# corelab-src/dacapo

Hardware: AMD Instinct MI355X
Metric: NTT/s (NTT-equivalents over one run() of the ResNet HEVM program, nt=2^14) (higher is better)
Workload: dtype u64; 1 GPU; ResNet-20 (SiLU) HEVM program traced from the reference's examples/benchmarks/ResNet.py with its resnet20.silu.model weights, nt=2^14 slots, N=2^15, 14 x 60-bit primes (SEAL_HEVM.cpp:39-53); one independent ciphertext stream per GPU; streams_per_gpu=1, parallelism=replicas x1 (no collective in the op path)

## Files before the change

### dacapo_amd/csrc/fused_ks.hip

```cpp
#include "ks_mac.hpp"

namespace dacapo {

struct SrcStrided {
    const u64 *base;
    long stride;
    int prime_base, period;
    __device__ int prime(int z) const { return prime_base + z % period; }
    __device__ u64 load(int z, int g, int) const { return base[(long)z * stride + g]; }
};
template <int E>
__device__ __forceinline__ void rs_operand(u64 (&v)[E], const int (&g)[E], const RsItem &it, const SumSrc *__restrict__ srcs, int p, int i,
                                           size_t N, const DModulus &M)
{
    if (it.count == 0) {
        const u64 *x = it.src.limb(p, i, N);
#pragma unroll
        for (int j = 0; j < E; j++) v[j] = x[g[j]];
    } else {
        u64 s[E];
        Acc128 a[E];
#pragma unroll
        for (int j = 0; j < E; j++) s[j] = 0, a[j].clear();
        int n_plain = 0, n_prod = 0;
// ... 173 lines not shown
                                                                              const DModulus *__restrict__ mods,
                                                                              const u64 *__restrict__ half_mod,
                                                                              const u64 *__restrict__ tw, const u64 *__restrict__ itw,
                                                                              int logN, const u64 *__restrict__ tw2)
{
    __shared__ __attribute__((aligned(16))) u64 lds[TileGeo<LOGE>::LDS_ELEMS];
    const int z = blockIdx.y, bp = MERGE ? z : z / cnt;
    const size_t N = (size_t)1 << logN;
    const u64 *in = last + (long)bp * last_stride;
    u64 x[1 << LOGE];
    auto nost = [](int, u64) {};
    ntt_tile_x<K, LOGE, true, true, true, false, true>(
        x, mods[l], itw + ((size_t)l << logN), logN, blockIdx.x, [=](int g) { return in[g]; }, nost, lds);
    const u64 ql = mods[l].q, half = ql >> 1;
#pragma unroll
    for (int r = 0; r < (1 << LOGE); r++) {
        const u64 y = x[r] + half;
        x[r] = y >= ql ? y - ql : y;
    }
    auto nold = [](int) -> u64 { return 0; };
    for (int i = MERGE ? 0 : z % cnt; i < (MERGE ? cnt : z % cnt + 1); i++) {
        u64 *out = tmp + ((size_t)bp * cnt + i) * N;
        const DModulus Mi = mods[i];
        const u64 qi = Mi.q, neg_half = qi - half_mod[(size_t)l * Kp + i];
        u64 y[1 << LOGE];
#pragma unroll
        for (int r = 0; r < (1 << LOGE); r++) {
            const u64 v = recanon(x[r], Mi) + neg_half;
            y[r] = v >= qi ? v - qi : v;
        }
        __syncthreads();
        ntt_tile_fcols<K, LOGE, false, true, false>(
            y, Mi, tw + ((size_t)i << logN), tw2 ? tw2 + ((size_t)i << (K + 1)) : nullptr, logN, blockIdx.x, nold, [=](int g, u64 v) { out[g] = v; }, lds);
    }
}

template <int K, int LOGE, bool MERGE>
__global__ __launch_bounds__(kTileThreads) void f_dr2_icols_lift_fcols_kernel(const u64 *__restrict__ acc, const MulRsItem *__restrict__ items,
                                                                               u64 *__restrict__ tmp, int ell, int Kp,
                                                                               const DModulus *__restrict__ mods,
                                                                               const u64 *__restrict__ half_mod,
                                                                               const u64 *__restrict__ inv_last, const u64 *__restrict__ tw,
                                                                               const u64 *__restrict__ itw, int logN, const u64 *__restrict__ tw2)
{
    __shared__ __attribute__((aligned(16))) u64 lds[TileGeo<LOGE>::LDS_ELEMS];
    constexpr int E = 1 << LOGE;
    const int cnt = ell - 1, L = ell - 1, sp = Kp - 1;
    const int z = blockIdx.y, bp = MERGE ? z : z / cnt;
    const size_t N = (size_t)1 << logN;
    const u64 *in_p = acc + ((size_t)bp * (ell + 1) + ell) * N, *in_l = acc + ((size_t)bp * (ell + 1) + L) * N;
    const u64 *mul = items[bp >> 1].mul;
    const long mul_stride = items[bp >> 1].mul_stride;
    auto nost = [](int, u64) {};
    u64 rho[E], u[E];
    ntt_tile_x<K, LOGE, true, true, true, false, true>(
        rho, mods[sp], itw + ((size_t)sp << logN), logN, blockIdx.x, [=](int g) { return in_p[g]; }, nost, lds);
    __syncthreads();
    const DModulus ML = mods[L];
    ntt_tile_x<K, LOGE, true, true, true, false, true>(
        u, ML, itw + ((size_t)L << logN), logN, blockIdx.x, [=](int g) { return in_l[g]; }, nost, lds);
    {
        const u64 P = mods[sp].q, half_p = P >> 1, qL = ML.q, half_l = qL >> 1;
        const u64 neg_half = qL - half_mod[(size_t)sp * Kp + L];
        u64 k = inv_last[(size_t)sp * Kp + L];
        if (mul) k = mulmod(mul[(long)L * mul_stride], k, ML);
#pragma unroll
// ... 727 lines not shown
#define DC_MERGED_LAUNCH(limbs, sources, per_source, KERNEL, ...)                                                                          \
    {                                                                                                                                     \
        const bool tiny = use_tiny_tiles(c.N, (limbs)), small = !tiny && use_small_tiles(c.N, (limbs));                                  \
        const int le = tiny ? 1 : small ? 2 : 3;                                                                                          \
        const bool merge = (per_source) > 1 && (long)(c.N >> (le == 1 ? TileGeo<1>::LOG : le == 2 ? TileGeo<2>::LOG : TileGeo<3>::LOG)) * (sources) >= ks_merge_lift_min_wgs(); \
        if (!merge) {                                                                                                                     \
            DC_GEO_SWITCH(c.k1, (limbs), DC_LAUNCH((KERNEL<KK, LE, false>), grid, dim3(kTileThreads), 0, s, __VA_ARGS__));      \
        } else if (le == 1) {                                                                                                             \
            constexpr int LE = 1;                                                                                                         \
            const dim3 grid((unsigned)(c.N >> TileGeo<LE>::LOG), (unsigned)(sources));                                                    \
            DC_K_SWITCH(c.k1, DC_LAUNCH((KERNEL<KK, LE, true>), grid, dim3(kTileThreads), 0, s, __VA_ARGS__))                    \
        } else if (le == 2) {                                                                                                             \
            constexpr int LE = 2;                                                                                                         \
            const dim3 grid((unsigned)(c.N >> TileGeo<LE>::LOG), (unsigned)(sources));                                                    \
            DC_K_SWITCH(c.k1, DC_LAUNCH((KERNEL<KK, LE, true>), grid, dim3(kTileThreads), 0, s, __VA_ARGS__))                    \
        } else {                                                                                                                          \
            constexpr int LE = 3;                                                                                                         \
            const dim3 grid((unsigned)(c.N >> TileGeo<LE>::LOG), (unsigned)(sources));                                                    \
            DC_K_SWITCH(c.k1, DC_LAUNCH((KERNEL<KK, LE, true>), grid, dim3(kTileThreads), 0, s, __VA_ARGS__))                    \
        }                                                                                                                                 \
    }

void f_ks_icols_lift_fcols(const Context &c, const u64 *digits, u64 *ext, int B, int ell, hipStream_t s)
{
    DC_MERGED_LAUNCH(B * ell * ell, B * ell, ell, f_ks_icols_lift_fcols_kernel, digits, ext, ell, c.K - 1, c.d_mods, c.d_tw, c.d_itw, c.logN, c.twc2())
}

void f_dr_icols_lift_fcols(const Context &c, const u64 *last, long last_stride, u64 *tmp, int polys, int cnt, int l, hipStream_t s)
{
    DC_MERGED_LAUNCH(polys * cnt, polys, cnt, f_dr_icols_lift_fcols_kernel, last, last_stride, tmp, cnt, l, c.K, c.d_mods, c.d_half_mod, c.d_tw,
                     c.d_itw, c.logN, c.twc2())
}

void f_dr2_icols_lift_fcols(const Context &c, const u64 *acc, const MulRsItem *items, u64 *tmp, int B, int ell, hipStream_t s)
{
    DC_MERGED_LAUNCH(2 * B * (ell - 1), 2 * B, ell - 1, f_dr2_icols_lift_fcols_kernel, acc, items, tmp, ell, c.K, c.d_mods, c.d_half_mod, c.d_inv_last,
                     c.d_tw, c.d_itw, c.logN, c.twc2())
}
#undef DC_MERGED_LAUNCH

void f_frows_fold_final(const Context &c, const u64 *tmp, const MulRsItem *items, const u64 *acc, int B, int ell, hipStream_t s, const Handoff &h)
{
    const int cnt = ell - 1, groups = h.cont == CONT_BOOT ? B : 2 * B;
#define DC_FOLD(CT)                                                                                                                    \
    DC_GEO_SWITCH(c.k2, groups * cnt, DC_LAUNCH((f_frows_fold_final_kernel<KK, LE, CT>), grid, dim3(kTileThreads), 0, s, tmp, items, acc, ell, c.K, \
                                                         c.d_mods, c.d_inv_last, c.d_tw, c.d_itw, c.logN, h))
    switch (h.cont) {
    case CONT_NONE: DC_FOLD(CONT_NONE); break;
    case CONT_MUL: DC_FOLD(CONT_MUL); break;
    case CONT_BOOT: DC_FOLD(CONT_BOOT); break;
    default: fprintf(stderr, "[dacapo_amd] f_frows_fold_final: no continuation kernel for consumer kind %d\n", h.cont); abort();
    }
#undef DC_FOLD
}

void f_ks_lift_fcols(const Context &c, const u64 *digits, u64 *ext, int B, int ell, hipStream_t s)
{
    if ((c.k1 == 7 || c.k1 == 8) && use_wide_tiles(c.N, (long)B * ell * ell) && !use_small_tiles(c.N, (long)B * ell * ell)) {
        constexpr int LE = 4;
        const dim3 grid((unsigned)(c.N >> TileGeo<LE>::LOG), (unsigned)(B * ell * ell));
        if (c.k1 == 7)
            DC_LAUNCH((f_ks_lift_fcols_kernel<7, LE>), grid, dim3(kTileThreads), 0, s, digits, ext, ell, c.K - 1, c.d_mods, c.d_tw, c.logN, c.twc2());
        else
            DC_LAUNCH((f_ks_lift_fcols_kernel<8, LE>), grid, dim3(kTileThreads), 0, s, digits, ext, ell, c.K - 1, c.d_mods, c.d_tw, c.logN, c.twc2());
        return;
    }
// ... 49 lines not shown
```

### dacapo_amd/csrc/hevm_vm.hip

```cpp
#include "hevm_vm.hpp"

#include "../../include/dacapo_ckks.h"
#include "c_api_types.hpp"
#include "chacha.hpp"
#include "seal_serial.hpp"

#include <math.h>
#include <string.h>
#include <sys/random.h>

#include <algorithm>
#include <cmath>
#include <chrono>
#include <fstream>
#include <iostream>

namespace dacapo {

constexpr int kVmThreads = 256;

constexpr int kRngCoefs = 8;

__device__ __forceinline__ int rng_cbd(u64 w)
{
// ... 33 lines not shown
            if (r[e] >= q) r[e] = w[e] >> sh;
    }
    u64x2 *o = reinterpret_cast<u64x2 *>(out + (size_t)i * N + blk * kRngCoefs);
#pragma unroll
    for (int e = 0; e < kRngCoefs; e += 2) o[e >> 1] = u64x2{ r[e], r[e + 1] };
}

__global__ __launch_bounds__(kVmThreads) void sample_small_kernel(u64 *__restrict__ out, size_t N, int limbs, int cbd, ChaChaKey key,
                                                                   u64 object, u32 domain, const DModulus *__restrict__ mods)
{
    const size_t blk = (size_t)blockIdx.x * kVmThreads + threadIdx.x;
    u64 w[kRngCoefs];
    rng_words8(key, object, blk, 0, 0, domain, w);
    int v[kRngCoefs];
#pragma unroll
    for (int e = 0; e < kRngCoefs; e++) v[e] = cbd ? rng_cbd(w[e]) : rng_ternary(w[e]);
    for (int i = 0; i < limbs; i++) store_small8(out + (size_t)i * N + blk * kRngCoefs, v, mods[i].q);
}

__global__ __launch_bounds__(kVmThreads) void sample_enc_batch_kernel(u64 *__restrict__ out, size_t N, int cnt, ChaChaKey key, u64 object0,
                                                                       const DModulus *__restrict__ mods,
                                                                       const u64 *__restrict__ epoch)
{
    const int b = blockIdx.y / 3, z = blockIdx.y % 3;
    const size_t blk = (size_t)blockIdx.x * kVmThreads + threadIdx.x;
    u64 w[kRngCoefs];
    rng_words8(key, object0 + (u64)b, blk, *epoch, 0, RNG_ENC_U + (u32)z, w);
    int v[kRngCoefs];
#pragma unroll
    for (int e = 0; e < kRngCoefs; e++) v[e] = z ? rng_cbd(w[e]) : rng_ternary(w[e]);
    for (int i = 0; i < cnt; i++) store_small8(out + (((size_t)b * 3 + z) * cnt + i) * N + blk * kRngCoefs, v, mods[i].q);
}

__global__ void chacha_blocks_kernel(u32 *__restrict__ out, ChaChaKey key, u64 counter, u64 nonce, int blocks)
{
    const int b = blockIdx.x * blockDim.x + threadIdx.x;
    if (b >= blocks) return;
    u32 o[16];
    chacha20_block(key, counter + (u64)b, nonce, o);
    for (int i = 0; i < 16; i++) out[b * 16 + i] = o[i];
}

__global__ void bump_epoch_kernel(u64 *epoch) { *epoch += 1; }

__global__ __launch_bounds__(kVmThreads) void lift_i128_kernel(u64 *__restrict__ out, const u64 *__restrict__ lo,
                                                                const u64 *__restrict__ hi, size_t N,
                                                                const DModulus *__restrict__ mods)
{
    const int i = blockIdx.y;
    const DModulus M = mods[i];
    const size_t k = (size_t)blockIdx.x * kVmThreads + threadIdx.x;
    u64 l = lo[k], h = hi[k];
    const bool neg = (h >> 63) != 0;
    if (neg) {
        l = ~l + 1;
        h = ~h + (l == 0);
    }
    const u64 r = reduce128_any(h, l, M);
    out[(size_t)i * N + k] = neg ? negmod(r, M.q) : r;
}

__global__ __launch_bounds__(kVmThreads) void ezs_final_kernel(u64 *__restrict__ c0, const u64 *__restrict__ c1,
                                                                const u64 *__restrict__ sk, const u64 *__restrict__ newkey,
                                                                int digit_lo, int digit_hi, const u64 *__restrict__ pmod, size_t N,
                                                                const DModulus *__restrict__ mods)
{
// ... 241 lines not shown
    int ksp = std::max(1, (int)option(OPT_KS_SPECIAL));
    int alpha = option(OPT_KS_ALPHA) > 0 ? (int)option(OPT_KS_ALPHA) : ksp;
    if (dir_ksp > 0) {
        if ((ksp != 1 || alpha != 1) && (ksp != dir_ksp || alpha != dir_alpha)) {
            fprintf(stderr, "[dacapo_amd] the key directory was written with ks_special = %d, ks_alpha = %d; options ask for %d / %d\n", dir_ksp,
                    dir_alpha, ksp, alpha);
            abort();
        }
        ksp = dir_ksp, alpha = dir_alpha;
    }
    ks_hoist = option(OPT_KS_HOIST) != 0;
    if (ks_hoist && (ksp > 1 || alpha > 1)) {
        fprintf(stderr, "[dacapo_amd] option ks_hoist = 1 is for SEAL-layout keys (ks_special = 1); with ks_special = %d, ks_alpha = %d key switching uses "
                        "grouped digits, which already shares a source's decomposition among its hops\n", ksp, alpha);
        abort();
    }
    ks_lazy = (int)option(OPT_KS_LAZY_SUM);
    if (ks_lazy && (ksp > 1 || alpha > 1)) {
        fprintf(stderr, "[dacapo_amd] option ks_lazy_sum = %d is for SEAL-layout keys (ks_special = 1); with ks_special = %d, ks_alpha = %d the lazy sums "
                        "of grouped-digit key switching are options hyb_lazy_sum / hyb_double_hoist\n", ks_lazy, ksp, alpha);
        abort();
    }
    if (ks_lazy && !ks_hoist) {
        fprintf(stderr, "[dacapo_amd] option ks_lazy_sum = %d needs ks_hoist = 1: a lazy sum is defined on digits taken before the automorphism "
                        "(ks_hoist = 0 here)\n", ks_lazy);
        abort();
    }
    ks_fold_rescale = option(OPT_KS_FOLD_RESCALE) != 0;
    if (ks_fold_rescale && (ksp > 1 || alpha > 1)) {
        fprintf(stderr, "[dacapo_amd] option ks_fold_rescale = 1 is for SEAL-layout keys (ks_special = 1); with ks_special = %d, ks_alpha = %d the mod-down "
                        "is an approximate base conversion, and dividing by P q in one exact pass does not reproduce it\n", ksp, alpha);
        abort();
    }
    const int bits = (int)option(OPT_PRIME_BITS);
    ctx.reset(new Context(logN, K, bits, primes, ksp, alpha));
    ctx->ensure_scratch();
    encoder.reset(new HostEncoder(logN));
    use_plan = option(OPT_PLAN) != 0;
    plan_graph = option(OPT_PLAN_GRAPH) != 0;
    plan_dag = option(OPT_PLAN_GRAPH) == 2;
    plan_lanes = option(OPT_PLAN_LANES) >= 2 ? 2 : 1;
    host_encoder = option(OPT_HOST_ENCODER) != 0;
    fold_rescale_into_boot = option(OPT_FOLD_RESCALE_BOOT) != 0;
    lazy_sums = option(OPT_HYB_LAZY_SUM) != 0;
    double_hoist = (lazy_sums && option(OPT_HYB_DOUBLE_HOIST) != 0) || ks_lazy == 2;
    max_batch = std::max(1, (int)option(OPT_MAX_BATCH));
    chain_fusion = option(OPT_CHAIN_FUSION) != 0;
    secret_weight = (int)option(OPT_SECRET_HW);
    boot_secret_weight = (int)option(OPT_BOOT_SECRET_HW);
    rot_compose = option(OPT_ROT_COMPOSE) != 0;
    online_encode = option(OPT_ONLINE_ENCODE) != 0 && use_plan && !host_encoder;
    lanes.resize(1);
    DC_HIP_CHECK(hipStreamCreateWithFlags(&lanes[0].stream, hipStreamNonBlocking));
    lanes[0].ws = ctx->ws0;
    lanes[0].boot_plain.d = dalloc((size_t)ctx->max_level() * ctx->N);
    lanes[0].boot_plain.level = ctx->max_level();
    DC_HIP_CHECK(vm_malloc(&d_epoch, 8));
    DC_HIP_CHECK(hipMemset(d_epoch, 0, 8));
    cur = 0;
}

void HEVM::gen_kswitch_key(u64 *key, const u64 *new_key, u64 key_id) { gen_kswitch_key_in(*ctx, key, keys.sk, new_key, key_id); }

void HEVM::gen_kswitch_key_in(Context &c, u64 *key, const u64 *key_sk, const u64 *new_key, u64 key_id)
{
    const size_t N = c.N;
// ... 1215 lines not shown
{
    Context &c = *ctx;
    const size_t N = c.N;
    if (!keys.sk || !keys.pk || ell < 1 || target_level < 1 || target_level > c.max_level()) {
        fprintf(stderr, "[dacapo_amd] bootstrap: needs a full VM (secret + public key) and a valid target level\n");
        abort();
    }
    const double new_scale = pow(2.0, (double)(int64_t)std::log2(src_scale));
    const CrtTables &tb = crt_tables(ell);
    u64 *pt = W().ks_tmp;
    u64 *lohi = W().ks_digits;
    f_irows_decrypt(c, src, keys.sk, ell, pt, S());
    launch_ntt_cols_inv(c, pt, (long)N, ell, nullptr, 0, 0, S());
    const CrtDev cd{ tb.inv, tb.mmod, tb.hmod, tb.hdig, tb.mdbl };
    DC_LAUNCH(reencode_kernel, dim3((unsigned)((N / 2 + kVmThreads) / kVmThreads)), dim3(kVmThreads), 0, S(), lohi,
                       lohi + N, pt, ell, N, c.d_mods, cd, new_scale / src_scale);
    Plain ptx{ lanes[cur].boot_plain.d, target_level, new_scale };
    DC_LAUNCH(lift_i128_kernel, dim3((unsigned)(N / kVmThreads), (unsigned)target_level), dim3(kVmThreads), 0, S(),
                       ptx.d, lohi, lohi + N, N, c.d_mods);
    launch_ntt(c, false, ptx.d, (long)N, target_level, nullptr, 0, 0, S());
    encrypt_plain(dst, ptx);
}

void HEVM::plan_zero_encrypt(int first, int B, int t, hipStream_t s)
{
    Context &c = *ctx;
    const size_t N = c.N;
    const int cnt = t + 1;
    if (!keys.pk) {
        fprintf(stderr, "[dacapo_amd] bootstrap: this VM has no public key\n");
        abort();
    }
    Plan &P = plan;
    DC_LAUNCH(sample_enc_batch_kernel, dim3((unsigned)(N / (kRngCoefs * kVmThreads)), (unsigned)(3 * B)), dim3(kVmThreads), 0, s,
                       P.boot_ue, N, cnt, rng.secret, ((u64)1 << 32) + (u64)first, c.d_mods, d_epoch);
    launch_ntt(c, false, P.boot_ue, (long)N, 3 * cnt * B, nullptr, 0, cnt, s);
    DC_LAUNCH(pk_encrypt_batch_kernel, dim3((unsigned)(N / (2 * kVmThreads)), (unsigned)cnt, (unsigned)(2 * B)), dim3(kVmThreads),
                       0, s, P.boot_tmp, keys.pk, (long)c.K * (long)N, P.boot_ue, cnt, N, c.d_mods);
    b_rescale(c, P.ws[0], P.d_boot_rs + first, B, cnt, s);
}

void HEVM::plan_boot_step(int first, int B, int ell, int t, int lane, hipStream_t s, const Handoff &h)
{
    Context &c = *ctx;
    const size_t N = c.N;
    if (!keys.sk) {
        fprintf(stderr, "[dacapo_amd] bootstrap: needs a full VM (secret + public key)\n");
        abort();
    }
    Plan &P = plan;
    const BootItem *items = P.d_boot + first;
    const CrtTables &tb = crt_tables(ell);
    const CrtDev cd{ tb.inv, tb.mmod, tb.hmod, tb.hdig, tb.mdbl };
    u64 *pt = P.boot_pt[lane], *ptx = P.boot_ptx[lane];
    if (h.in)
        pt = const_cast<u64 *>(h.in);
    else
        f_irows_decrypt_items(c, items, P.d_sum_srcs, keys.sk, ell, pt, B, s);
    launch_ntt_cols_inv(c, pt, (long)N, B * ell, nullptr, 0, ell, s);
    if (ell == 1)
        f_boot_reencode_fcols(c, pt, ptx, items, B, ell, t, cd, s);
    else {
        DC_LAUNCH(reencode_lift_batch_kernel, dim3((unsigned)((N / 2 + kVmThreads) / kVmThreads), (unsigned)B), dim3(kVmThreads), 0,
                           s, ptx, pt, items, ell, t, N, c.d_mods, cd);
        launch_ntt_cols_fwd(c, ptx, (long)N, B * t, nullptr, 0, t, s);
    }
// ... 436 lines not shown
```

### dacapo_amd/csrc/hevm_vm.hpp

```cpp
#pragma once
#include "wire_parse.hpp"
#include <complex>
#include <deque>
#include <map>
#include <set>
#include <memory>
#include <string>
#include <unordered_set>
#include <vector>

#include "../../include/hevm_abi.h"
#include "chacha.hpp"
#include "seal_serial.hpp"
#include "kernels.hpp"
#include "encoder.hpp"
#include "plan.hpp"

namespace dacapo {

struct VmAllocs {
    std::unordered_set<void *> live;
};
extern thread_local VmAllocs *g_vm_allocs;
template <class T>
// ... 141 lines not shown
        bool fold_rs = false;
        int gfirst = 0, gcount = 0;
        int unique = 0;
        std::vector<const u64 *> reads, writes;
    };
    struct Plan {
        bool ready = false;
        std::vector<Val> vals;
        std::vector<Pop> pops;
        std::vector<Step> steps;
        std::vector<int> final_val;
        KsItem *d_ks = nullptr;
        MulItem *d_mul = nullptr;
        MulRsItem *d_mulrs = nullptr;
        RsItem *d_rs = nullptr;
        EwItem *d_ew = nullptr;
        SumItem *d_sum = nullptr;
        SumSrc *d_sum_srcs = nullptr;
        SumGroup *d_sumg = nullptr;
        SumGroupSrc *d_sumg_srcs = nullptr;
        CtView *d_cont_other = nullptr;
        struct EncGroup { int wave, level, first, count; u64 *out; };
        std::vector<EncGroup> enc_groups;
        EncItem *d_enc_items = nullptr;
        u64 *enc_arena = nullptr;
        double2 *enc_scratch = nullptr;
        int *d_enc_overflow = nullptr;
        size_t enc_arena_bytes = 0, enc_scratch_bytes = 0;
        std::vector<EwItem> h_ew;
        std::vector<u64 *> handoff_bufs;
        size_t n_fused = 0;
        BootItem *d_boot = nullptr;
        RsItem *d_boot_rs = nullptr;
        size_t zenc_bytes = 0;
        u64 *zenc = nullptr, *boot_ue = nullptr, *boot_tmp = nullptr, *boot_pt[2] = { nullptr, nullptr }, *boot_ptx[2] = { nullptr, nullptr };
        struct BootChunk { int first, count, target; };
        std::vector<BootChunk> boot_chunks;
        BatchWs ws[2];
        std::vector<hipEvent_t> events;
        std::vector<u64 *> pool;
        int64_t n_keyswitch = 0, n_ntt = 0;
        int64_t n_hops = 0, n_decomp = 0;
        int64_t n_fold = 0;
        size_t launches = 0, max_live = 0;
        hipGraph_t graph = nullptr;
        hipGraphExec_t graph_exec = nullptr;
    } plan;
    bool plan_graph = true;
    bool plan_dag = false;
    void capture_plan();
    bool capture_plan_dag();
    void issue_step(const Step &st, hipStream_t q);
    void drop_plan_graph();
    void issue_plan(hipStream_t s);
    bool use_plan = true;
    bool test_zero_enc = false;
    int max_batch = 64;
    std::vector<u64 *> home;
    int streams = 1, sel = 0;
    std::vector<u64 *> reg_base;
    void set_streams(int n);
    void select_stream(int s);
    void build_plan();
    void run_plan();
    void boot_item(CtView src, int src_level, double src_scale, hevm_ctxt &dst, int target_level);
    void plan_zero_encrypt(int first, int B, int t, hipStream_t s);
    void plan_boot_step(int first, int B, int ell, int t, int lane, hipStream_t s, const Handoff &h);
    bool rot_compose = false;
    std::vector<int> compose_rotation(int steps) const;
    mutable std::vector<int> rot_offsets;
    mutable std::set<int> rot_offset_set;
    mutable size_t rot_offsets_epoch = (size_t)-1;
    int boot_secret_weight = 0;
    int secret_weight = 0;
    bool ks_hoist = false;
    int ks_lazy = 0;
    bool ks_fold_rescale = false;
    KsItem *d_hoist_items = nullptr;
    void rotate_hop_vm(CtView dst, CtView src, u32 elt, const u64 *key, int ell);
    bool chain_fusion = true;
    hipStream_t aux_stream = nullptr;
    bool double_hoist = false;
    double *dh_consts = nullptr;
    std::map<int, EncItem> dh_items;
    void ensure_special_limbs(const std::vector<int> &plain_regs);
    bool lazy_sums = false;
    bool fold_rescale_into_boot = false;
    int plan_lanes = 2;
    void bump_epoch(hipStream_t s);

    int64_t op_counts[11] = { 0 };
    int64_t n_keyswitch = 0, n_ntt = 0;
    int64_t n_hops = 0, n_decomp = 0;
    int64_t n_fold = 0;
    double t_bootstrap = 0.0;

    VmAllocs allocs;
    HEVM() { g_vm_allocs = &allocs; }
    void destroy_device_state();
    size_t key_elems() const { return (size_t)ctx->key_digits() * 2 * ctx->K * ctx->N; }
    void init_context(int logN, int K, const u64 *primes, int dir_ksp = 0, int dir_alpha = 0);
    void generate_keys(const RngKeys &rng, bool secret, bool pub, bool eval);
    void gen_kswitch_key(u64 *key, const u64 *new_key, u64 key_id);
    void gen_kswitch_key_in(Context &c, u64 *key, const u64 *key_sk, const u64 *new_key, u64 key_id);
    void fill_sparse_secret(u64 *dst, int weight, u32 domain);
    void generate_boot_switch_keys();
    size_t swk_down_elems() const { return (size_t)2 * (1 + ctx->ksp) * ctx->N; }
    void add_galois_key(u32 elt);
    void save_keys(const std::string &dir);
    void load_keys(const std::string &dir, bool need_secret, bool need_public, bool need_eval);
// ... 36 lines not shown
```

### dacapo_amd/csrc/options.cpp

```cpp
#include "options.hpp"

#include "../../include/hevm_abi.h"

#include <stdio.h>
#include <stdlib.h>
#include <string.h>

namespace dacapo {

struct OptDef {
    const char *name;
    long long def;
};
static const OptDef kDefs[OPT_COUNT] = {
    { "logn", 15 },
    { "primes", 14 },
    { "prime_bits", 60 },
    { "ks_special", 1 },
    { "ks_alpha", 0 },
    { "secret_hw", 0 },
    { "boot_secret_hw", 0 },
    { "rot_compose", 0 },
    { "plan", 1 },
    { "plan_graph", 1 },
    { "plan_lanes", 2 },
    { "plan_aux_min_cost", 3 },
    { "max_batch", 64 },
    { "chain_fusion", 1 },
    { "host_encoder", 0 },
    { "online_encode", 0 },
    { "fold_rescale_boot", 0 },
    { "hyb_mfma", 1 },
    { "hyb_fuse", 2 },
    { "hyb_lazy_sum", 0 },
    { "hyb_double_hoist", 0 },
    { "ks_hoist", 0 },
    { "ks_lazy_sum", 0 },
    { "ks_fold_rescale", 0 },
    { "seal_compr", 0 },
    { "trace", 0 },
    { "step_profile", 0 },
    { "small_tile_wgs", -1 },
    { "tiny_tile_wgs", 2000 },
    { "wide_tile_wgs", 2048 },
    { "rows_prime_major", 16 },
    { "ntt_full_min_limbs", 768 },
    { "ntt_full_inv_min_limbs", 768 },
    { "ntt_full_persist", -1 },
    { "ntt_full_inv_persist", -1 },
    { "ntt_full_pairs", 1 },
    { "ntt_full_inv_pairs", 1 },
    { "cols_pairs", 1 },
    { "ks_merge_special_min_wgs", 2048 },
    { "ks_merge_lift_min_wgs", 1024 },
    { "ks_items_fast", 1 },
    { "ks_fuse_mac", 1 },
    { "ks_big_tiles", 4096 },
    { "ks_fuse_mac_tiles", 1LL << 40 },
    { "sum_pair_min_wgs", 1024 },
    { "sum_group_min_wgs", 2048 },
};

static long long g_val[OPT_COUNT];
static bool g_init = false;

static int find(const char *name, size_t len)
{
    for (int i = 0; i < OPT_COUNT; i++)
        if (strlen(kDefs[i].name) == len && !strncmp(kDefs[i].name, name, len)) return i;
    return -1;
}
// ... 100 lines not shown
```

### dacapo_amd/csrc/options.hpp

```cpp
#pragma once

namespace dacapo {

enum Opt : int {
    OPT_LOGN,
    OPT_PRIMES,
    OPT_PRIME_BITS,
    OPT_KS_SPECIAL,
    OPT_KS_ALPHA,
    OPT_SECRET_HW,
    OPT_BOOT_SECRET_HW,
    OPT_ROT_COMPOSE,
    OPT_PLAN,
    OPT_PLAN_GRAPH,
    OPT_PLAN_LANES,
    OPT_PLAN_AUX_MIN_COST,
    OPT_MAX_BATCH,
    OPT_CHAIN_FUSION,
    OPT_HOST_ENCODER,
    OPT_ONLINE_ENCODE,
    OPT_FOLD_RESCALE_BOOT,
    OPT_HYB_MFMA,
    OPT_HYB_FUSE,
    OPT_HYB_LAZY_SUM,
    OPT_HYB_DOUBLE_HOIST,
    OPT_KS_HOIST,
    OPT_KS_LAZY_SUM,
    OPT_KS_FOLD_RESCALE,
    OPT_SEAL_COMPR,
    OPT_TRACE,
    OPT_STEP_PROFILE,
    OPT_SMALL_TILE_WGS,
    OPT_TINY_TILE_WGS,
    OPT_WIDE_TILE_WGS,
    OPT_ROWS_PRIME_MAJOR,
    OPT_NTT_FULL_MIN_LIMBS,
    OPT_NTT_FULL_INV_MIN_LIMBS,
    OPT_NTT_FULL_PERSIST,
    OPT_NTT_FULL_INV_PERSIST,
    OPT_NTT_FULL_PAIRS,
    OPT_NTT_FULL_INV_PAIRS,
    OPT_COLS_PAIRS,
    OPT_KS_MERGE_SPECIAL_MIN_WGS,
    OPT_KS_MERGE_LIFT_MIN_WGS,
    OPT_KS_ITEMS_FAST,
    OPT_KS_FUSE_MAC,
    OPT_KS_BIG_TILES,
    OPT_KS_FUSE_MAC_TILES,
    OPT_SUM_PAIR_MIN_WGS,
    OPT_SUM_GROUP_MIN_WGS,
    OPT_COUNT
};

long long option(Opt o);

}
```

### dacapo_amd/csrc/plan.hpp

```cpp
#pragma once
#include "crt_device.hpp"
#include "kernels.hpp"

namespace dacapo {

struct KsItem {
    CtView src, dst;
    const u64 *key;
    u32 elt;
    u32 slot;
    const u64 *plain = nullptr, *plain_sp = nullptr;
};
struct MulItem {
    CtView a, b, dst;
};
struct MulRsItem : MulItem {
    const u64 *add = nullptr;
    const u64 *mul = nullptr;
    long mul_stride = 0;
};
struct RsItem {
    CtView src, dst;
    int first = 0, count = 0;
    const u64 *add = nullptr;
    const u64 *mul = nullptr;
};
struct EwItem {
    CtView dst, a, b;
};
struct SumSrc {
    CtView v;
    const u64 *plain;
};
struct SumItem {
    CtView dst;
    int first, count;
};

constexpr int kSumGroup = 8;
struct SumGroupSrc {
    CtView v;
    const u64 *plain[kSumGroup];
};
struct SumGroup {
    CtView dst[kSumGroup];
    int first, count, items;
};
__host__ __device__ inline const u64 *sum_add_only() { return reinterpret_cast<const u64 *>((uintptr_t)8); }

struct BootItem {
    CtView src, dst;
    const u64 *zenc;
    double ratio;
    int first = 0, count = 0;
    const u64 *add = nullptr, *mul = nullptr;
};

enum ContKind : int {
// ... 37 lines not shown
void hyb_rotate_hop_single(Context &c, const Workspace &w, CtView dst, CtView src, u32 galois_elt, const u64 *galois_key, int ell, hipStream_t s);
void hyb_mul_relin(Context &c, const BatchWs &w, const MulItem *d_items, const u64 *relin_key, int B, int ell, hipStream_t s);
void hyb_keyswitch(Context &c, const Workspace &w, CtView out, const u64 *base0, const u64 *base1, const u64 *target, const u64 *key, int ell,
                   hipStream_t s);
inline int64_t ks_ntt_count(const Context &c, int ell)
{
    return c.hybrid() ? (int64_t)c.hyb_groups(ell) * (ell + c.ksp) + 2 * c.ksp + 2 * ell : (int64_t)(ell + 1) * (ell + 2);
}
void b_ew(Context &c, EwOp op, const EwItem *d_items, int B, int polys, int b_polys, int ell, hipStream_t s);
void b_add_plain(Context &c, const EwItem *d_items, int B, int ell, hipStream_t s);
void b_sum(Context &c, const SumItem *d_items, const SumSrc *d_srcs, int B, int ell, hipStream_t s);
void b_sum_group(Context &c, const SumGroup *d_groups, const SumGroupSrc *d_gsrcs, int G, int ell, hipStream_t s);
void modraise(Context &c, u64 *scratch, const EwItem *h_items, int B, int target, hipStream_t s, const EwItem *d_items = nullptr);

void f_irows_strided(const Context &c, const u64 *base, long stride, int prime_base, int period, u64 *out, long out_stride, int count,
                     hipStream_t s);
void f_irows_rot_c1(const Context &c, const KsItem *items, int ell, u64 *out, int B, hipStream_t s);
void f_irows_rs_last(const Context &c, const RsItem *items, const SumSrc *srcs, int l, u64 *out, int B, hipStream_t s);
void f_irows_rs_single(const Context &c, CtView src, int l, u64 *out, hipStream_t s);
void f_irows_decrypt(const Context &c, CtView ct, const u64 *sk, int ell, u64 *out, hipStream_t s);
void f_irows_tensor_c2(const Context &c, const MulItem *items, int ell, u64 *out, int B, hipStream_t s);
void f_irows_decrypt_items(const Context &c, const BootItem *items, const SumSrc *srcs, const u64 *sk, int ell, u64 *out, int B,
                           hipStream_t s);
void f_irows_tensor_c2_rs(const Context &c, const MulRsItem *items, int ell, u64 *out, int B, hipStream_t s);
void f_ks_frows_mac_rs(const Context &c, const u64 *ext, const MulRsItem *items, const u64 *relin_key, u64 *acc, int B, int ell, hipStream_t s);
void f_dr2_icols_lift_fcols(const Context &c, const u64 *acc, const MulRsItem *items, u64 *tmp, int B, int ell, hipStream_t s);
void f_frows_fold_final(const Context &c, const u64 *tmp, const MulRsItem *items, const u64 *acc, int B, int ell, hipStream_t s,
                        const Handoff &h = Handoff{});
void f_boot_reencode_fcols(const Context &c, const u64 *pt, u64 *ptx, const BootItem *items, int B, int ell, int t, CrtDev crt,
                           hipStream_t s);
void f_frows_boot_final(const Context &c, const u64 *ptx, const BootItem *items, int B, int t, hipStream_t s);
void f_ks_icols_lift_fcols(const Context &c, const u64 *digits, u64 *ext, int B, int ell, hipStream_t s);
void f_dr_icols_lift_fcols(const Context &c, const u64 *last, long last_stride, u64 *tmp, int polys, int cnt, int l, hipStream_t s);
void f_ks_frows_mac(const Context &c, int mode, const u64 *ext, const u64 *target, const KsItem *items, const u64 *shared_key, u64 *acc,
                    int B, int ell, hipStream_t s, bool fold_base = false);
void f_ks_lift_fcols(const Context &c, const u64 *digits, u64 *ext, int B, int ell, hipStream_t s);
void f_dr_lift_fcols(const Context &c, const u64 *last, long last_stride, u64 *tmp, int polys, int cnt, int l, hipStream_t s);
void f_frows_final(const Context &c, int mode, const u64 *tmp, const void *items, const u64 *acc, int polys, int cnt, int l,
                   hipStream_t s, RsItem single = RsItem{}, const u64 *plain = nullptr, const SumSrc *srcs = nullptr,
                   const Handoff &h = Handoff{}, bool base_folded = false);
void fill_const_plain(Context &c, u64 *out, const u64 *d_residues, int ell, hipStream_t s);
void rescale_fused(Context &c, const Workspace &w, CtView dst, CtView src, int ell, const u64 *plain, hipStream_t s);

}
```

### dacapo_amd/csrc/plan_exec.hip

```cpp
#include <math.h>
#include <string.h>

#include <algorithm>
#include <chrono>
#include <map>
#include <functional>
#include <queue>
#include <set>
#include <tuple>

#include "hevm_vm.hpp"

namespace dacapo {

#define ks_ntts(ell) ks_ntt_count(c, (ell))

template <class T>
static T *upload(const std::vector<T> &v)
{
    T *d = nullptr;
    DC_HIP_CHECK(vm_malloc(&d, std::max<size_t>(v.size(), 1) * sizeof(T)));
    if (!v.empty()) DC_HIP_CHECK(hipMemcpy(d, v.data(), v.size() * sizeof(T), hipMemcpyHostToDevice));
    return d;
}

void HEVM::build_plan()
{
    Context &c = *ctx;
    const size_t N = c.N;
    Plan &P = plan;
    for (u64 *b : P.handoff_bufs) (void)vm_free(b);
    P.handoff_bufs.clear();
    for (void *p : { (void *)P.d_enc_items, (void *)P.enc_arena, (void *)P.enc_scratch, (void *)P.d_enc_overflow })
        if (p) (void)vm_free(p);
    P.d_enc_items = nullptr, P.enc_arena = nullptr, P.enc_scratch = nullptr, P.d_enc_overflow = nullptr;
    P.enc_groups.clear(), P.enc_arena_bytes = P.enc_scratch_bytes = 0;
    if (P.d_cont_other) (void)vm_free(P.d_cont_other), P.d_cont_other = nullptr;
    if (P.d_mulrs) (void)vm_free(P.d_mulrs), P.d_mulrs = nullptr;
    for (void *p : { (void *)P.d_ks, (void *)P.d_mul, (void *)P.d_rs, (void *)P.d_ew, (void *)P.d_sum, (void *)P.d_sum_srcs, (void *)P.d_sumg, (void *)P.d_sumg_srcs, (void *)P.d_boot,
                     (void *)P.d_boot_rs, (void *)P.zenc, (void *)P.boot_ue, (void *)P.boot_tmp, (void *)P.boot_pt[0], (void *)P.boot_ptx[0],
                     (void *)P.boot_pt[1], (void *)P.boot_ptx[1] })
        if (p) (void)vm_free(p);
    P.d_boot = nullptr, P.d_boot_rs = nullptr, P.zenc = P.boot_ue = P.boot_tmp = nullptr;
    P.boot_pt[0] = P.boot_pt[1] = P.boot_ptx[0] = P.boot_ptx[1] = nullptr;
    P.boot_chunks.clear();
    if (P.graph_exec) (void)hipGraphExecDestroy(P.graph_exec);
    if (P.graph) (void)hipGraphDestroy(P.graph);
    P.graph_exec = nullptr, P.graph = nullptr;
    P.vals.clear(), P.pops.clear(), P.steps.clear();
    P.n_keyswitch = P.n_ntt = 0;
    P.n_hops = P.n_decomp = 0, P.n_fold = 0;
    const size_t nreg = ciphers.size();
    const int S = streams;
    std::vector<int> cur(nreg, -1);
    auto new_val = [&](int level, double scale) {
        Val v;
        v.level = level, v.scale = scale, v.root = (int)P.vals.size();
        P.vals.push_back(v);
        return (int)P.vals.size() - 1;
    };
    auto need = [&](int r, const char *what) {
        if (r < 0 || (size_t)r >= nreg || cur[(size_t)r] < 0) {
            fprintf(stderr, "[dacapo_amd] %s reads cipher register %d before anything wrote it\n", what, r);
            abort();
        }
        return cur[(size_t)r];
    };
    auto add_pop = [&](PopKind k, int level, std::vector<int> srcs, int dst) -> Pop & {
        Pop p;
        p.kind = k, p.level = level, p.srcs = std::move(srcs), p.dst = dst;
        P.vals[(size_t)dst].def_pop = (int)P.pops.size();
        P.pops.push_back(p);
        return P.pops.back();
    };
    for (size_t i = 0; i < header.arg_length; i++) {
        const int v = new_val((int)arg_level[i], pow(2.0, (double)arg_scale[i]));
// ... 898 lines not shown
        } else if (st.kind == P_RESCALE) {
            need_d = std::max(need_d, B * 2), need_m = std::max(need_m, B * 2 * l);
            P.launches += 3;
        } else
            P.launches += st.kind == P_BOOT ? 5 : 1;
    }
    for (size_t s = 0; s < P.steps.size(); s++) {
        Step &st = P.steps[s];
        st.reads.clear(), st.writes.clear();
        for (int pi : step_pops[s]) {
            const Pop &p = O[(size_t)pi];
            for (int v : p.srcs) st.reads.push_back(V[(size_t)V[(size_t)v].root].buf);
            st.writes.push_back(V[(size_t)V[(size_t)p.dst].root].buf);
        }
        if (st.fold_rs)
            for (int pi : fold_pops.at(s)) st.writes.push_back(V[(size_t)V[(size_t)O[(size_t)pi].dst].root].buf);
        if (st.fused_consumer >= 0 && st.h.cont == CONT_MUL)
            for (int pi : step_pops[(size_t)st.fused_consumer])
                for (int v : O[(size_t)pi].srcs) st.reads.push_back(V[(size_t)V[(size_t)v].root].buf);
        for (auto *vec : { &st.reads, &st.writes }) {
            std::sort(vec->begin(), vec->end());
            vec->erase(std::unique(vec->begin(), vec->end()), vec->end());
        }
    }
    if (!h_boot_pops.empty()) {
        const size_t nb = h_boot_pops.size(), slot = (size_t)2 * boot_tmax * N;
        DC_HIP_CHECK(vm_malloc(&P.zenc, nb * slot * sizeof(u64)));
        P.zenc_bytes = nb * slot * sizeof(u64);
        std::vector<int> order(nb);
        for (size_t i = 0; i < nb; i++) order[i] = (int)i;
        std::stable_sort(order.begin(), order.end(), [&](int a, int b) {
            return O[(size_t)h_boot_pops[(size_t)a].first].target_level < O[(size_t)h_boot_pops[(size_t)b].first].target_level;
        });
        const size_t bc = std::min<size_t>(nb, (size_t)std::max(max_batch, 1));
        const size_t cmax = (size_t)boot_tmax + 1;
        DC_HIP_CHECK(vm_malloc(&P.boot_ue, bc * 3 * cmax * N * sizeof(u64)));
        DC_HIP_CHECK(vm_malloc(&P.boot_tmp, bc * 2 * cmax * N * sizeof(u64)));
        for (int ln = 0; ln < plan_lanes; ln++) {
            DC_HIP_CHECK(vm_malloc(&P.boot_pt[ln], std::max<size_t>(need_bpt, 1) * N * sizeof(u64)));
            DC_HIP_CHECK(vm_malloc(&P.boot_ptx[ln], std::max<size_t>(need_bptx, 1) * N * sizeof(u64)));
        }
        std::vector<BootItem> h_boot(nb);
        std::vector<RsItem> h_brs(nb);
        for (size_t k = 0; k < nb;) {
            const int t = O[(size_t)h_boot_pops[(size_t)order[k]].first].target_level;
            size_t e = k;
            while (e < nb && e - k < bc && O[(size_t)h_boot_pops[(size_t)order[e]].first].target_level == t) e++;
            P.boot_chunks.push_back({ (int)k, (int)(e - k), t });
            for (size_t j = k; j < e; j++) {
                const size_t item = (size_t)order[j];
                u64 *z = P.zenc + item * slot;
                h_brs[j] = RsItem{ CtView{ P.boot_tmp + (j - k) * 2 * (size_t)(t + 1) * N, (long)(t + 1) * (long)N }, CtView{ z, (long)t * (long)N } };
            }
            need_d = std::max(need_d, (e - k) * 2), need_m = std::max(need_m, (e - k) * 2 * (size_t)(t + 1));
            P.launches += 7;
            k = e;
        }
        for (size_t item = 0; item < nb; item++) {
            const Pop &p = O[(size_t)h_boot_pops[item].first];
            const int q = h_boot_pops[item].second;
            const double new_scale = V[(size_t)p.dst].scale;
            BootItem bi{ view(p.srcs[0], q), view(p.dst, q), P.zenc + item * slot, 1.0 };
            double src_scale;
            if (p.boot_drop >= 0) {
                src_scale = p.boot_src_scale * (double)c.primes[(size_t)p.boot_drop];
            } else
                src_scale = V[(size_t)p.srcs[0]].scale;
            bi.ratio = new_scale / src_scale;
            if (p.rs_sum) {
                bi.first = (int)h_srcs.size(), bi.count = (int)p.srcs.size();
                for (size_t k = 0; k < p.srcs.size(); k++) {
                    const int pl = p.src_plain.empty() ? -1 : p.src_plain[k];
                    h_srcs.push_back(SumSrc{ view(p.srcs[k], q), pl >= 0 ? plains.at((size_t)pl).d : nullptr });
                }
            }
            if (p.rs_add >= 0) bi.add = plains.at((size_t)p.rs_add).d;
            if (p.rs_mul >= 0) bi.mul = plains.at((size_t)p.rs_mul).d;
            h_boot[item] = bi;
        }
        P.d_boot = upload(h_boot), P.d_boot_rs = upload(h_brs);
    }
    P.d_mulrs = upload(h_mulrs);
    P.d_ks = upload(h_ks), P.d_mul = upload(h_mul), P.d_rs = upload(h_rs), P.d_ew = upload(h_ew), P.d_sum = upload(h_sum);
    P.h_ew = h_ew;
    P.d_sum_srcs = upload(h_srcs);
    P.d_sumg = upload(h_sumg), P.d_sumg_srcs = upload(h_sumg_srcs);
    {
        std::vector<size_t> other_first(P.steps.size(), 0);
        for (size_t ai = 0; ai < P.steps.size(); ai++) {
            Step &A = P.steps[ai];
            if (A.fused_consumer < 0) continue;
            Step &B = P.steps[(size_t)A.fused_consumer];
            const size_t items = (size_t)B.count, limbs = A.h.cont == CONT_RS ? 2 : (size_t)B.level;
            u64 *buf = nullptr;
            DC_HIP_CHECK(vm_malloc(&buf, items * limbs * N * sizeof(u64)));
            P.handoff_bufs.push_back(buf);
            A.h.out = buf, B.h.in = buf;
            A.h.sk = keys.sk;
            if (A.h.cont == CONT_RS) A.h.rs_items = P.d_rs + B.first;
            if (A.h.cont == CONT_MUL) {
                other_first[ai] = h_cont_other.size();
                for (int pi : step_pops[(size_t)A.fused_consumer])
                    for (int q = 0; q < S; q++) {
                        const Pop &mp = O[(size_t)pi];
                        const int w = mul_fused_src[(size_t)pi], other = mp.srcs[(size_t)(1 - w)];
                        h_cont_other.push_back(other == mp.srcs[(size_t)w] ? CtView{ nullptr, 0 } : view(other, q));
                    }
            }
        }
        P.d_cont_other = upload(h_cont_other);
        for (size_t ai = 0; ai < P.steps.size(); ai++)
            if (P.steps[ai].fused_consumer >= 0 && P.steps[ai].h.cont == CONT_MUL) P.steps[ai].h.other = P.d_cont_other + other_first[ai];
    }
// ... 369 lines not shown
```

Baseline: 1.266 million NTT/s.

## Fuse boot zero-encryption head: skip full-basis noise NTTs, fold drop-last into public-key product

Adds a zenc_head path, on by default, for generating the zero-encryptions used in bootstrapping. Only the u polynomial is sampled and NTT'd. The two error polynomials are kept as packed int8 in coefficient form and added inside a fused inverse-NTT / lift / forward-NTT drop-last kernel. The final kernel recomputes u*pk per limb and folds the subtraction and inv_last scaling, which removes the separate error NTTs, the boot_tmp buffer and one launch. The boot chunk size is fixed at 64 instead of max_batch, which changes batching and scratch sizing and risks a different launch count.

```diff
diff --git a/dacapo_amd/csrc/fused_ks.hip b/dacapo_amd/csrc/fused_ks.hip
--- a/dacapo_amd/csrc/fused_ks.hip
+++ b/dacapo_amd/csrc/fused_ks.hip
@@ -229,6 +229,108 @@
         __syncthreads();
         ntt_tile_fcols<K, LOGE, false, true, false>(
             y, Mi, tw + ((size_t)i << logN), tw2 ? tw2 + ((size_t)i << (K + 1)) : nullptr, logN, blockIdx.x, nold, [=](int g, u64 v) { out[g] = v; }, lds);
+    }
+}
+
+template <int K, int LOGE>
+__global__ __launch_bounds__(kTileThreads) void f_irows_zenc_kernel(const ZencItem *__restrict__ items, const u64 *__restrict__ pk, long pk_ps,
+                                                                     int l, u64 *__restrict__ out, const DModulus *__restrict__ mods,
+                                                                     const u64 *__restrict__ itw, int logN)
+{
+    __shared__ __attribute__((aligned(16))) u64 lds[TileGeo<LOGE>::LDS_ELEMS];
+    constexpr int E = 1 << LOGE;
+    const int z = blockIdx.y;
+    const size_t N = (size_t)1 << logN;
+    const DModulus M = mods[l];
+    u64 *o = out + (size_t)z * N;
+    const int g0 = tile_gidx<K, LOGE, false>(num_passes<LOGE>(K) - 1, logN, blockIdx.x, 0);
+    const u64 *u = items[z >> 1].u + (size_t)l * N + g0, *k = pk + (z & 1) * pk_ps + (size_t)l * N + g0;
+    u64 x[E];
+#pragma unroll
+    for (int j = 0; j < E; j += 2) {
+        const u64x2 a = *reinterpret_cast<const u64x2 *>(u + j), b = *reinterpret_cast<const u64x2 *>(k + j);
+        x[j] = mulmod(a.x, b.x, M), x[j + 1] = mulmod(a.y, b.y, M);
+    }
+    auto nold = [](int) -> u64 { return 0; };
+    ntt_tile_x<K, LOGE, false, true, false, true, false>(x, M, itw + ((size_t)l << logN), logN, blockIdx.x, nold,
+                                                         [=](int gi, u64 v) { o[gi] = v; }, lds);
+}
+
+template <int K, int LOGE, bool MERGE>
+__global__ __launch_bounds__(kTileThreads) void f_dr_noise_icols_lift_fcols_kernel(const u64 *__restrict__ last, long last_stride,
+                                                                                    u64 *__restrict__ tmp, int cnt, int l, int Kp,
+                                                                                    const DModulus *__restrict__ mods,
+                                                                                    const u64 *__restrict__ half_mod,
+                                                                                    const u64 *__restrict__ tw, const u64 *__restrict__ itw,
+                                                                                    int logN, const u64 *__restrict__ tw2,
+                                                                                    const signed char *__restrict__ noise)
+{
+    __shared__ __attribute__((aligned(16))) u64 lds[TileGeo<LOGE>::LDS_ELEMS];
+    const int z = blockIdx.y, bp = MERGE ? z : z / cnt;
+    const size_t N = (size_t)1 << logN;
+    const u64 *in = last + (long)bp * last_stride;
+    const signed char *ep = noise + (size_t)bp * N;
+    u64 x[1 << LOGE];
+    int e[1 << LOGE];
+#pragma unroll
+    for (int r = 0; r < (1 << LOGE); r++) e[r] = ep[tile_gidx<K, LOGE, true>(0, logN, blockIdx.x, r)];
+    auto nost = [](int, u64) {};
+    ntt_tile_x<K, LOGE, true, true, true, false, true>(
+        x, mods[l], itw + ((size_t)l << logN), logN, blockIdx.x, [=](int g) { return in[g]; }, nost, lds);
+    const u64 ql = mods[l].q, half = ql >> 1;
+#pragma unroll
+    for (int r = 0; r < (1 << LOGE); r++) {
+        u64 y = x[r] + (e[r] < 0 ? ql - (u64)(-e[r]) : (u64)e[r]);
+        y = y >= ql ? y - ql : y;
+        y += half;
+        x[r] = y >= ql ? y - ql : y;
+    }
+    auto nold = [](int) -> u64 { return 0; };
+    for (int i = MERGE ? 0 : z % cnt; i < (MERGE ? cnt : z % cnt + 1); i++) {
+        u64 *out = tmp + ((size_t)bp * cnt + i) * N;
+        const DModulus Mi = mods[i];
+        const u64 qi = Mi.q, neg_half = qi - half_mod[(size_t)l * Kp + i];
+        u64 y[1 << LOGE];
+#pragma unroll
+        for (int r = 0; r < (1 << LOGE); r++) {
+            u64 v = recanon(x[r], Mi) + neg_half;
+            v = v >= qi ? v - qi : v;
+            v += e[r] > 0 ? qi - (u64)e[r] : (u64)(-e[r]);
+            y[r] = v >= qi ? v - qi : v;
+        }
+        __syncthreads();
+        ntt_tile_fcols<K, LOGE, false, true, false>(
+            y, Mi, tw + ((size_t)i << logN), tw2 ? tw2 + ((size_t)i << (K + 1)) : nullptr, logN, blockIdx.x, nold, [=](int g, u64 v) { out[g] = v; }, lds);
+    }
+}
+
+template <int K, int LOGE>
+__global__ __launch_bounds__(kTileThreads) void f_frows_zenc_final_kernel(const u64 *__restrict__ tmp, const ZencItem *__restrict__ items,
+                                                                           const u64 *__restrict__ pk, long pk_ps, int l, int Kp,
+                                                                           const DModulus *__restrict__ mods,
+                                                                           const u64 *__restrict__ inv_last, const u64 *__restrict__ tw,
+                                                                           int logN)
+{
+    __shared__ __attribute__((aligned(16))) u64 lds[TileGeo<LOGE>::LDS_ELEMS];
+    constexpr int E = 1 << LOGE;
+    const int z = blockIdx.y, i = z % l, bp = z / l, b = bp >> 1, p = bp & 1;
+    const size_t N = (size_t)1 << logN;
+    const DModulus M = mods[i];
+    const u64 inv = inv_last[(size_t)l * Kp + i];
+    const u64 *in = tmp + (size_t)z * N;
+    const ZencItem it = items[b];
+    const int g0 = tile_gidx<K, LOGE, false>(num_passes<LOGE>(K) - 1, logN, blockIdx.x, 0);
+    const u64 *u = it.u + (size_t)i * N + g0, *k = pk + p * pk_ps + (size_t)i * N + g0;
+    u64 *o = it.dst.limb(p, i, N) + g0;
+    u64 v[E];
+    auto nost = [](int, u64) {};
+    ntt_tile_x<K, LOGE, false, false, true, false, true>(v, M, tw + ((size_t)i << logN), logN, blockIdx.x, [=](int gi) { return in[gi]; }, nost, lds);
+#pragma unroll
+    for (int j = 0; j < E; j += 2) {
+        const u64x2 a = *reinterpret_cast<const u64x2 *>(u + j), c = *reinterpret_cast<const u64x2 *>(k + j);
+        u64x2 r;
+        r.x = mulmod(submod(mulmod(a.x, c.x, M), v[j], M.q), inv, M), r.y = mulmod(submod(mulmod(a.y, c.y, M), v[j + 1], M.q), inv, M);
+        *reinterpret_cast<u64x2 *>(o + j) = r;
     }
 }
 
@@ -1022,6 +1124,23 @@
                      c.d_itw, c.logN, c.twc2())
 }
 
+void f_irows_zenc(const Context &c, const ZencItem *items, const u64 *pk, int l, u64 *out, int B, hipStream_t s)
+{
+    DC_GEO_SWITCH(c.k2, 2 * B, DC_LAUNCH((f_irows_zenc_kernel<KK, LE>), grid, dim3(kTileThreads), 0, s, items, pk, (long)c.K * (long)c.N, l, out,
+                                                  c.d_mods, c.d_itw, c.logN));
+}
+void f_dr_noise_icols_lift_fcols(const Context &c, const u64 *last, long last_stride, u64 *tmp, int polys, int cnt, int l,
+                                 const signed char *noise, hipStream_t s)
+{
+    DC_MERGED_LAUNCH(polys * cnt, polys, cnt, f_dr_noise_icols_lift_fcols_kernel, last, last_stride, tmp, cnt, l, c.K, c.d_mods, c.d_half_mod,
+                     c.d_tw, c.d_itw, c.logN, c.twc2(), noise)
+}
+void f_frows_zenc_final(const Context &c, const u64 *tmp, const ZencItem *items, const u64 *pk, int B, int l, hipStream_t s)
+{
+    DC_GEO_SWITCH(c.k2, 2 * B * l, DC_LAUNCH((f_frows_zenc_final_kernel<KK, LE>), grid, dim3(kTileThreads), 0, s, tmp, items, pk,
+                                                      (long)c.K * (long)c.N, l, c.K, c.d_mods, c.d_inv_last, c.d_tw, c.logN));
+}
+
 void f_dr2_icols_lift_fcols(const Context &c, const u64 *acc, const MulRsItem *items, u64 *tmp, int B, int ell, hipStream_t s)
 {
     DC_MERGED_LAUNCH(2 * B * (ell - 1), 2 * B, ell - 1, f_dr2_icols_lift_fcols_kernel, acc, items, tmp, ell, c.K, c.d_mods, c.d_half_mod, c.d_inv_last,
diff --git a/dacapo_amd/csrc/hevm_vm.hip b/dacapo_amd/csrc/hevm_vm.hip
--- a/dacapo_amd/csrc/hevm_vm.hip
+++ b/dacapo_amd/csrc/hevm_vm.hip
@@ -89,6 +89,28 @@
     for (int i = 0; i < cnt; i++) store_small8(out + (((size_t)b * 3 + z) * cnt + i) * N + blk * kRngCoefs, v, mods[i].q);
 }
 
+__global__ __launch_bounds__(kVmThreads) void sample_zenc_batch_kernel(u64 *__restrict__ u, signed char *__restrict__ e, size_t N, int cnt,
+                                                                        ChaChaKey key, u64 object0, const DModulus *__restrict__ mods,
+                                                                        const u64 *__restrict__ epoch)
+{
+    const int b = blockIdx.y / 3, z = blockIdx.y % 3;
+    const size_t blk = (size_t)blockIdx.x * kVmThreads + threadIdx.x;
+    u64 w[kRngCoefs];
+    rng_words8(key, object0 + (u64)b, blk, *epoch, 0, RNG_ENC_U + (u32)z, w);
+    int v[kRngCoefs];
+#pragma unroll
+    for (int k = 0; k < kRngCoefs; k++) v[k] = z ? rng_cbd(w[k]) : rng_ternary(w[k]);
+    if (z == 0) {
+        for (int i = 0; i < cnt; i++) store_small8(u + ((size_t)b * cnt + i) * N + blk * kRngCoefs, v, mods[i].q);
+    } else {
+        static_assert(kRngCoefs == 8, "one 8-byte store per thread");
+        u64 packed = 0;
+#pragma unroll
+        for (int k = 0; k < kRngCoefs; k++) packed |= (u64)(unsigned char)(signed char)v[k] << (8 * k);
+        *reinterpret_cast<u64 *>(e + ((size_t)b * 2 + (z - 1)) * N + blk * kRngCoefs) = packed;
+    }
+}
+
 __global__ void chacha_blocks_kernel(u32 *__restrict__ out, ChaChaKey key, u64 counter, u64 nonce, int blocks)
 {
     const int b = blockIdx.x * blockDim.x + threadIdx.x;
@@ -396,6 +418,7 @@
                         "is an approximate base conversion, and dividing by P q in one exact pass does not reproduce it\n", ksp, alpha);
         abort();
     }
+    zenc_head = option(OPT_ZENC_HEAD) != 0;
     const int bits = (int)option(OPT_PRIME_BITS);
     ctx.reset(new Context(logN, K, bits, primes, ksp, alpha));
     ctx->ensure_scratch();
@@ -1677,6 +1700,16 @@
         abort();
     }
     Plan &P = plan;
+    if (zenc_head) {
+        DC_LAUNCH(sample_zenc_batch_kernel, dim3((unsigned)(N / (kRngCoefs * kVmThreads)), (unsigned)(3 * B)), dim3(kVmThreads), 0, s,
+                           P.boot_ue, P.boot_e, N, cnt, rng.secret, ((u64)1 << 32) + (u64)first, c.d_mods, d_epoch);
+        launch_ntt(c, false, P.boot_ue, (long)N, cnt * B, nullptr, 0, cnt, s);
+        const ZencItem *items = P.d_boot_zenc + first;
+        f_irows_zenc(c, items, keys.pk, t, P.ws[0].digits, B, s);
+        f_dr_noise_icols_lift_fcols(c, P.ws[0].digits, (long)N, P.ws[0].tmp, 2 * B, t, t, P.boot_e, s);
+        f_frows_zenc_final(c, P.ws[0].tmp, items, keys.pk, B, t, s);
+        return;
+    }
     DC_LAUNCH(sample_enc_batch_kernel, dim3((unsigned)(N / (kRngCoefs * kVmThreads)), (unsigned)(3 * B)), dim3(kVmThreads), 0, s,
                        P.boot_ue, N, cnt, rng.secret, ((u64)1 << 32) + (u64)first, c.d_mods, d_epoch);
     launch_ntt(c, false, P.boot_ue, (long)N, 3 * cnt * B, nullptr, 0, cnt, s);
diff --git a/dacapo_amd/csrc/hevm_vm.hpp b/dacapo_amd/csrc/hevm_vm.hpp
--- a/dacapo_amd/csrc/hevm_vm.hpp
+++ b/dacapo_amd/csrc/hevm_vm.hpp
@@ -197,8 +197,10 @@
         size_t n_fused = 0;
         BootItem *d_boot = nullptr;
         RsItem *d_boot_rs = nullptr;
+        ZencItem *d_boot_zenc = nullptr;
         size_t zenc_bytes = 0;
         u64 *zenc = nullptr, *boot_ue = nullptr, *boot_tmp = nullptr, *boot_pt[2] = { nullptr, nullptr }, *boot_ptx[2] = { nullptr, nullptr };
+        signed char *boot_e = nullptr;
         struct BootChunk { int first, count, target; };
         std::vector<BootChunk> boot_chunks;
         BatchWs ws[2];
@@ -241,6 +243,9 @@
     bool ks_hoist = false;
     int ks_lazy = 0;
     bool ks_fold_rescale = false;
+    bool zenc_head = true;
+    static constexpr int kZencChunk = 64;
+    int zenc_chunk_hook = 0;
     KsItem *d_hoist_items = nullptr;
     void rotate_hop_vm(CtView dst, CtView src, u32 elt, const u64 *key, int ell);
     bool chain_fusion = true;
diff --git a/dacapo_amd/csrc/options.cpp b/dacapo_amd/csrc/options.cpp
--- a/dacapo_amd/csrc/options.cpp
+++ b/dacapo_amd/csrc/options.cpp
@@ -37,6 +37,7 @@
     { "ks_hoist", 0 },
     { "ks_lazy_sum", 0 },
     { "ks_fold_rescale", 0 },
+    { "zenc_head", 1 },
     { "seal_compr", 0 },
     { "trace", 0 },
     { "step_profile", 0 },
diff --git a/dacapo_amd/csrc/options.hpp b/dacapo_amd/csrc/options.hpp
--- a/dacapo_amd/csrc/options.hpp
+++ b/dacapo_amd/csrc/options.hpp
@@ -27,6 +27,7 @@
     OPT_KS_HOIST,
     OPT_KS_LAZY_SUM,
     OPT_KS_FOLD_RESCALE,
+    OPT_ZENC_HEAD,
     OPT_SEAL_COMPR,
     OPT_TRACE,
     OPT_STEP_PROFILE,
diff --git a/dacapo_amd/csrc/plan.hpp b/dacapo_amd/csrc/plan.hpp
--- a/dacapo_amd/csrc/plan.hpp
+++ b/dacapo_amd/csrc/plan.hpp
@@ -24,6 +24,10 @@
     int first = 0, count = 0;
     const u64 *add = nullptr;
     const u64 *mul = nullptr;
+};
+struct ZencItem {
+    const u64 *u;
+    CtView dst;
 };
 struct EwItem {
     CtView dst, a, b;
@@ -127,6 +131,10 @@
 void f_frows_boot_final(const Context &c, const u64 *ptx, const BootItem *items, int B, int t, hipStream_t s);
 void f_ks_icols_lift_fcols(const Context &c, const u64 *digits, u64 *ext, int B, int ell, hipStream_t s);
 void f_dr_icols_lift_fcols(const Context &c, const u64 *last, long last_stride, u64 *tmp, int polys, int cnt, int l, hipStream_t s);
+void f_irows_zenc(const Context &c, const ZencItem *items, const u64 *pk, int l, u64 *out, int B, hipStream_t s);
+void f_dr_noise_icols_lift_fcols(const Context &c, const u64 *last, long last_stride, u64 *tmp, int polys, int cnt, int l,
+                                 const signed char *noise, hipStream_t s);
+void f_frows_zenc_final(const Context &c, const u64 *tmp, const ZencItem *items, const u64 *pk, int B, int l, hipStream_t s);
 void f_ks_frows_mac(const Context &c, int mode, const u64 *ext, const u64 *target, const KsItem *items, const u64 *shared_key, u64 *acc,
                     int B, int ell, hipStream_t s, bool fold_base = false);
 void f_ks_lift_fcols(const Context &c, const u64 *digits, u64 *ext, int B, int ell, hipStream_t s);
diff --git a/dacapo_amd/csrc/plan_exec.hip b/dacapo_amd/csrc/plan_exec.hip
--- a/dacapo_amd/csrc/plan_exec.hip
+++ b/dacapo_amd/csrc/plan_exec.hip
@@ -38,10 +38,10 @@
     if (P.d_cont_other) (void)vm_free(P.d_cont_other), P.d_cont_other = nullptr;
     if (P.d_mulrs) (void)vm_free(P.d_mulrs), P.d_mulrs = nullptr;
     for (void *p : { (void *)P.d_ks, (void *)P.d_mul, (void *)P.d_rs, (void *)P.d_ew, (void *)P.d_sum, (void *)P.d_sum_srcs, (void *)P.d_sumg, (void *)P.d_sumg_srcs, (void *)P.d_boot,
-                     (void *)P.d_boot_rs, (void *)P.zenc, (void *)P.boot_ue, (void *)P.boot_tmp, (void *)P.boot_pt[0], (void *)P.boot_ptx[0],
+                     (void *)P.d_boot_rs, (void *)P.d_boot_zenc, (void *)P.zenc, (void *)P.boot_ue, (void *)P.boot_tmp, (void *)P.boot_pt[0], (void *)P.boot_ptx[0],
                      (void *)P.boot_pt[1], (void *)P.boot_ptx[1] })
         if (p) (void)vm_free(p);
-    P.d_boot = nullptr, P.d_boot_rs = nullptr, P.zenc = P.boot_ue = P.boot_tmp = nullptr;
+    P.d_boot = nullptr, P.d_boot_rs = nullptr, P.d_boot_zenc = nullptr, P.zenc = P.boot_ue = P.boot_tmp = nullptr, P.boot_e = nullptr;
     P.boot_pt[0] = P.boot_pt[1] = P.boot_ptx[0] = P.boot_ptx[1] = nullptr;
     P.boot_chunks.clear();
     if (P.graph_exec) (void)hipGraphExecDestroy(P.graph_exec);
@@ -1006,16 +1006,22 @@
         std::stable_sort(order.begin(), order.end(), [&](int a, int b) {
             return O[(size_t)h_boot_pops[(size_t)a].first].target_level < O[(size_t)h_boot_pops[(size_t)b].first].target_level;
         });
-        const size_t bc = std::min<size_t>(nb, (size_t)std::max(max_batch, 1));
+        const size_t bc = std::min<size_t>(nb, zenc_head ? (size_t)(zenc_chunk_hook > 0 ? zenc_chunk_hook : kZencChunk) : (size_t)std::max(max_batch, 1));
         const size_t cmax = (size_t)boot_tmax + 1;
-        DC_HIP_CHECK(vm_malloc(&P.boot_ue, bc * 3 * cmax * N * sizeof(u64)));
-        DC_HIP_CHECK(vm_malloc(&P.boot_tmp, bc * 2 * cmax * N * sizeof(u64)));
+        if (zenc_head) {
+            DC_HIP_CHECK(vm_malloc(&P.boot_ue, bc * cmax * N * sizeof(u64) + bc * 2 * N));
+            P.boot_e = reinterpret_cast<signed char *>(P.boot_ue + bc * cmax * N);
+        } else {
+            DC_HIP_CHECK(vm_malloc(&P.boot_ue, bc * 3 * cmax * N * sizeof(u64)));
+            DC_HIP_CHECK(vm_malloc(&P.boot_tmp, bc * 2 * cmax * N * sizeof(u64)));
+        }
         for (int ln = 0; ln < plan_lanes; ln++) {
             DC_HIP_CHECK(vm_malloc(&P.boot_pt[ln], std::max<size_t>(need_bpt, 1) * N * sizeof(u64)));
             DC_HIP_CHECK(vm_malloc(&P.boot_ptx[ln], std::max<size_t>(need_bptx, 1) * N * sizeof(u64)));
         }
         std::vector<BootItem> h_boot(nb);
-        std::vector<RsItem> h_brs(nb);
+        std::vector<RsItem> h_brs(zenc_head ? 0 : nb);
+        std::vector<ZencItem> h_bz(zenc_head ? nb : 0);
         for (size_t k = 0; k < nb;) {
             const int t = O[(size_t)h_boot_pops[(size_t)order[k]].first].target_level;
             size_t e = k;
@@ -1024,10 +1030,13 @@
             for (size_t j = k; j < e; j++) {
                 const size_t item = (size_t)order[j];
                 u64 *z = P.zenc + item * slot;
-                h_brs[j] = RsItem{ CtView{ P.boot_tmp + (j - k) * 2 * (size_t)(t + 1) * N, (long)(t + 1) * (long)N }, CtView{ z, (long)t * (long)N } };
-            }
-            need_d = std::max(need_d, (e - k) * 2), need_m = std::max(need_m, (e - k) * 2 * (size_t)(t + 1));
-            P.launches += 7;
+                if (zenc_head)
+                    h_bz[j] = ZencItem{ P.boot_ue + (j - k) * (size_t)(t + 1) * N, CtView{ z, (long)t * (long)N } };
+                else
+                    h_brs[j] = RsItem{ CtView{ P.boot_tmp + (j - k) * 2 * (size_t)(t + 1) * N, (long)(t + 1) * (long)N }, CtView{ z, (long)t * (long)N } };
+            }
+            need_d = std::max(need_d, (e - k) * 2), need_m = std::max(need_m, (e - k) * 2 * (size_t)(zenc_head ? t : t + 1));
+            P.launches += zenc_head ? 6 : 7;
             k = e;
         }
         for (size_t item = 0; item < nb; item++) {
@@ -1052,7 +1061,7 @@
             if (p.rs_mul >= 0) bi.mul = plains.at((size_t)p.rs_mul).d;
             h_boot[item] = bi;
         }
-        P.d_boot = upload(h_boot), P.d_boot_rs = upload(h_brs);
+        P.d_boot = upload(h_boot), P.d_boot_rs = upload(h_brs), P.d_boot_zenc = upload(h_bz);
     }
     P.d_mulrs = upload(h_mulrs);
     P.d_ks = upload(h_ks), P.d_mul = upload(h_mul), P.d_rs = upload(h_rs), P.d_ew = upload(h_ew), P.d_sum = upload(h_sum);
```

New measurement: 1.310 million NTT/s (median of 6 runs). 3.5% higher.
